# aminrezaee/mujoco_reinforcement_learning

Hardware: AMD Instinct MI355X
Metric: env-steps/sec (whole node) HalfCheetah-v4 4096 envs at 1/2/4/8 MI355X (higher is better)
Workload: dtype bf16; 1 GPU; HalfCheetah-v4 shapes: 4096 envs/GPU x 128 steps, obs 17, act 6, actor+critic 256x256 ReLU MLP, PPO 10 epochs x 8 minibatches of 65536; num_envs_per_gpu=4096, horizon=128, minibatch=65536, epochs=10, rng=philox, hipgraphs=True, env=device (synthetic dynamics on the GPU), parallelism=dp1 (env-sharded, RCCL grad all-reduce)

## Files before the change

### mujoco_reinforcement_learning_amd/csrc/fused_update.h

```cpp
#pragma once

#include <hip/hip_runtime.h>

#include <cstdint>

#include "ppo_loss.h"
#include "reduce_slabs.h"
#include "timing.h"

namespace ppo {

constexpr int kFusedRows = 64;
constexpr int kFusedKX = 32;
constexpr int kFusedSP = 16;
constexpr int kFusedMaxAct = 8;
constexpr int kFusedMaxWG = 128;
constexpr int kStampSlots = 13;

struct FusedNet {
  const __bf16 *w0b;
  const __bf16 *w1b;
  const __bf16 *w1bt;
  const float *w0, *w1;
  const float *b0, *b1;
  const float *wh, *bh;
  int64_t off_w0, off_b0, off_w1, off_b1, off_wh, off_bh;
};

constexpr int kRecordBytes = 2 * kFusedKX + 4 * kFusedSP;
static_assert(kRecordBytes == 128, "one record per 128 B line");
int fused_records_launch(uint4 *rec, const float *states, const float *actions,
                         const float *old_logp, const float *adv, const float *vtarget,
                         int64_t n_rows, int din, int act_dim, const TimRec &trec, hipStream_t st);

struct GaeRecordArgs {
  const float *value, *next_value;
  const void *reward;
  const uint8_t *done, *term;
  int force_last, n, t_len;
  float gamma_f, lg_f;
  float *adv, *vtarget;
  const float *states, *actions, *old_logp;
  uint4 *rec;
  int din, act_dim;
};
int gae_records_launch(const GaeRecordArgs &g, bool reward_f64, const TimRec &rec,
                       hipStream_t st);

struct AdamPackArgs {
  float *p;
  const float *g;
  float *m, *v;
  int64_t n, n_actor;
  const float *sched;
  float neg_a, neg_c, bc2;
  float w1, b2, omb2, eps;
  __bf16 *w0b[2], *w1b[2], *w1bt[2];
  int64_t off_w0[2], off_w1[2];
  int din, H;
};
int adam_pack_launch(const AdamPackArgs &a, const TimRec &rec, hipStream_t st);

struct TailArgs {
  AdamPackArgs a;
  const int32_t *rows;
  const uint4 *rec;
  int64_t n_rec;
  __bf16 *xb;
  float *srow;
  int b;
  bool reduce;
};
int step_tail_launch(const ReduceArgs &r, const TailArgs &t, const TimRec &rec, hipStream_t st);

struct FusedArgs {
  FusedNet net[2];
  const float *logstd;
  int64_t off_logstd;
  __bf16 *xb;
  float *srow;
  const float *states, *actions, *old_logp, *adv, *vtarget;
  const int32_t *rows;
  const int32_t *rows_n;
  const uint4 *rec;
  int64_t n_rec;
  bool direct;
  bool pack_w;
  int b, din, act_dim, act, hidden;
  float omv;
  LossCoef coef;
  float *slabs;
  int64_t slab_stride;
  float *loss_part;
  int G;
  uint64_t *stamps;
};
int fused_prep_launch(const FusedArgs &q, const TimRec &rec, hipStream_t st);
int fused_update_launch(const FusedArgs &q, const TimRec &rec, hipStream_t st);
bool fused_width_ok(int hidden);
int fused_sched(int act);

}
```

### mujoco_reinforcement_learning_amd/csrc/fused_update.hip

```cpp
#include <cstdio>
#include <cstdlib>
#include <type_traits>

#include "adam_elem.h"
#include "fused_common.h"
#include "gae_pipe.h"

namespace ppo {

using namespace fu;

__device__ __forceinline__ uint16_t bf16_bits(float x) { return static_cast<uint16_t>(pack2(x, 0.f) & 0xffffu); }

__global__ __launch_bounds__(256) void fused_prep_kernel(FusedArgs q, int row_blocks) {
  const int tid = threadIdx.x;
  if (static_cast<int>(blockIdx.x) < row_blocks && q.rec) {
    const int j = static_cast<int>((static_cast<int64_t>(blockIdx.x) * 256 + tid) >> 3);
    const int u = tid & 7;
    if (j >= q.b) return;
    const int count = q.rows_n ? *q.rows_n : q.b;
    uint4 v = make_uint4(0u, 0u, 0u, 0u);
    if (j < count) {
      const int64_t sr = q.rows[j];
      if (sr >= 0 && sr < q.n_rec) v = q.rec[sr * (kRecordBytes / 16) + u];
// ... 111 lines not shown
      s[k] = k < A ? act[b][k] : (k == A ? lp[b] : (k == A + 1 ? ad : (k == A + 2 ? vt : 0.f)));
    uint4 *d = rec + row * (kRecordBytes / 16);
#pragma unroll
    for (int u = 0; u < kFusedKX / 8; ++u)
      d[u] = make_uint4(pack2(x[b][8 * u], x[b][8 * u + 1]), pack2(x[b][8 * u + 2], x[b][8 * u + 3]),
                        pack2(x[b][8 * u + 4], x[b][8 * u + 5]), pack2(x[b][8 * u + 6], x[b][8 * u + 7]));
#pragma unroll
    for (int u = 0; u < kFusedSP / 4; ++u)
      d[kFusedKX / 8 + u] = make_uint4(__float_as_uint(s[4 * u]), __float_as_uint(s[4 * u + 1]),
                                       __float_as_uint(s[4 * u + 2]), __float_as_uint(s[4 * u + 3]));
  }
};

template <typename RT, int EB, int KMAX>
__global__ __launch_bounds__(EB * 16) void gae_records_kernel(GaeRecordArgs g) {
  RecordEmit em;
  em.states = g.states;
  em.actions = g.actions;
  em.old_logp = g.old_logp;
  em.rec = g.rec;
  em.din = g.din;
  em.A = g.act_dim;
  gae_pipe_body<RT, EB, KMAX>(g.value, g.next_value, static_cast<const RT *>(g.reward), g.done,
                              g.term, g.force_last, g.n, g.t_len, g.gamma_f, g.lg_f, g.adv,
                              g.vtarget, em);
}

constexpr int kPackTile = 32;

__global__ __launch_bounds__(256) void adam_pack_kernel(AdamPackArgs a, int gen_blocks) {
  const float ns_a = a.sched ? a.sched[0] : a.neg_a;
  const float ns_c = a.sched ? a.sched[1] : a.neg_c;
  const float bc2 = a.sched ? a.sched[2] : a.bc2;
  const int tid = threadIdx.x;
  const int H = a.H;
  if (static_cast<int>(blockIdx.x) < gen_blocks) {
    const int64_t i = static_cast<int64_t>(blockIdx.x) * 256 + tid;
    if (i >= a.n) return;
#pragma unroll
    for (int z = 0; z < 2; ++z)
      if (i >= a.off_w1[z] && i < a.off_w1[z] + static_cast<int64_t>(H) * H) return;
    float m = a.m[i], v = a.v[i];
    const float p = adam_elem(a.p[i], a.g[i], m, v, i < a.n_actor ? ns_a : ns_c, a.w1, a.b2,
                              a.omb2, bc2, a.eps);
    a.p[i] = p;
    a.m[i] = m;
    a.v[i] = v;
#pragma unroll
    for (int z = 0; z < 2; ++z) {
      const int64_t e = i - a.off_w0[z];
      if (e >= 0 && e < static_cast<int64_t>(H) * a.din) {
        const int f = static_cast<int>(e / a.din), k = static_cast<int>(e % a.din);
        reinterpret_cast<uint16_t *>(a.w0b[z])[f * kFusedKX + k] = bf16_bits(p);
      }
    }
    return;
  }
  __shared__ uint16_t tile[kPackTile][kPackTile + 2];
  const int tiles = H / kPackTile;
  const int tb = static_cast<int>(blockIdx.x) - gen_blocks;
  const int z = tb / (tiles * tiles);
  const int to = (tb % (tiles * tiles)) / tiles, tc = tb % tiles;
  const int64_t base = a.off_w1[z];
  const float ns = base < a.n_actor ? ns_a : ns_c;
  uint16_t *w1b = reinterpret_cast<uint16_t *>(a.w1b[z]);
  uint16_t *w1bt = reinterpret_cast<uint16_t *>(a.w1bt[z]);
#pragma unroll 4
  for (int k = 0; k < kPackTile * kPackTile / 256; ++k) {
    const int idx = k * 256 + tid, lo = idx / kPackTile, lc = idx % kPackTile;
    const int64_t t = static_cast<int64_t>(to * kPackTile + lo) * H + tc * kPackTile + lc;
    const int64_t i = base + t;
    float m = a.m[i], v = a.v[i];
    const float p = adam_elem(a.p[i], a.g[i], m, v, ns, a.w1, a.b2, a.omb2, bc2, a.eps);
    a.p[i] = p;
    a.m[i] = m;
    a.v[i] = v;
    const uint16_t hb = bf16_bits(p);
    w1b[w_frag(to * kPackTile + lo, tc * kPackTile + lc, H)] = hb;
    tile[lo][lc] = hb;
  }
  __syncthreads();
#pragma unroll 4
  for (int k = 0; k < kPackTile * kPackTile / 256; ++k) {
    const int idx = k * 256 + tid, lc = idx / kPackTile, lo = idx % kPackTile;
    w1bt[w_frag(tc * kPackTile + lc, to * kPackTile + lo, H)] = tile[lo][lc];
  }
}

__device__ __forceinline__ void tail_gather(const TailArgs &t, int64_t idx) {
  const int j = static_cast<int>(idx >> 3);
  const int u = static_cast<int>(idx & 7);
  if (j >= t.b) return;
  const int64_t sr = t.rows[j];
  uint4 v = make_uint4(0u, 0u, 0u, 0u);
  if (sr >= 0 && sr < t.n_rec) v = t.rec[sr * (kRecordBytes / 16) + u];
  if (u < 4) reinterpret_cast<uint4 *>(t.xb + static_cast<int64_t>(j) * kFusedKX)[u] = v;
  else reinterpret_cast<uint4 *>(t.srow + static_cast<int64_t>(j) * kFusedSP)[u - 4] = v;
}

__device__ __forceinline__ void adam_apply(const AdamPackArgs &a, int64_t i, float4 g4, float4 p4,
                                           float4 m4, float4 v4) {
  const float ns = i < a.n_actor ? (a.sched ? a.sched[0] : a.neg_a) : (a.sched ? a.sched[1] : a.neg_c);
  const float bc2 = a.sched ? a.sched[2] : a.bc2;
  p4.x = adam_elem(p4.x, g4.x, m4.x, v4.x, ns, a.w1, a.b2, a.omb2, bc2, a.eps);
  p4.y = adam_elem(p4.y, g4.y, m4.y, v4.y, ns, a.w1, a.b2, a.omb2, bc2, a.eps);
  p4.z = adam_elem(p4.z, g4.z, m4.z, v4.z, ns, a.w1, a.b2, a.omb2, bc2, a.eps);
  p4.w = adam_elem(p4.w, g4.w, m4.w, v4.w, ns, a.w1, a.b2, a.omb2, bc2, a.eps);
  *reinterpret_cast<float4 *>(a.p + i) = p4;
  *reinterpret_cast<float4 *>(a.m + i) = m4;
  *reinterpret_cast<float4 *>(a.v + i) = v4;
  const float pv[4] = {p4.x, p4.y, p4.z, p4.w};
  const int H = a.H;
#pragma unroll
  for (int z = 0; z < 2; ++z) {
    const int64_t e1 = i - a.off_w1[z];
    if (e1 >= 0 && e1 < static_cast<int64_t>(H) * H) {
      const int o = static_cast<int>(e1 / H), c = static_cast<int>(e1 % H);
      *reinterpret_cast<uint2 *>(a.w1b[z] + w_frag(o, c, H)) = make_uint2(pack2(pv[0], pv[1]), pack2(pv[2], pv[3]));
      uint16_t *wt = reinterpret_cast<uint16_t *>(a.w1bt[z]);
#pragma unroll
      for (int e = 0; e < 4; ++e) wt[w_frag(c + e, o, H)] = bf16_bits(pv[e]);
    }
    const int64_t e0 = i - a.off_w0[z];
#pragma unroll
    for (int e = 0; e < 4; ++e) {
      if (e0 + e >= 0 && e0 + e < static_cast<int64_t>(H) * a.din) {
        const int f = static_cast<int>((e0 + e) / a.din), k = static_cast<int>((e0 + e) % a.din);
        reinterpret_cast<uint16_t *>(a.w0b[z])[f * kFusedKX + k] = bf16_bits(pv[e]);
      }
    }
  }
}

template <int G>
__device__ __forceinline__ void tail_block(const ReduceArgs &r, const TailArgs &t, int64_t blk,
                                           RedScratch sc) {
  const int tid = threadIdx.x;
  const AdamPackArgs &a = t.a;
  const int64_t i = blk * (4 * G) + 4 * (tid % G);
  const bool lead = tid < G;
  float4 g4;
  if (t.reduce) {
    g4 = reduce_slab_block_s<G>(r, blk, sc);
    if (!lead || i >= r.total) return;
  } else {
    if (!lead || i >= a.n) return;
    g4 = *reinterpret_cast<const float4 *>(a.g + i);
  }
  adam_apply(a, i, g4, *reinterpret_cast<const float4 *>(a.p + i),
             *reinterpret_cast<const float4 *>(a.m + i), *reinterpret_cast<const float4 *>(a.v + i));
}

template <int G>
__global__ __launch_bounds__(G * kRedChunks) void step_tail_kernel(ReduceArgs r, TailArgs t, int red_blocks) {
  __shared__ __attribute__((aligned(16))) char scratch[red_scratch_bytes<G>()];
  constexpr int NT = G * kRedChunks;
  const int tid = threadIdx.x;
  if (static_cast<int>(blockIdx.x) >= red_blocks) {
    tail_gather(t, (static_cast<int64_t>(blockIdx.x) - red_blocks) * NT + tid);
    return;
  }
  tail_block<G>(r, t, blockIdx.x, red_scratch<G>(scratch));
}

template <int H, bool F32A2>
struct Lds {
  static constexpr int PITCH = 2 * H;
  static constexpr int A2P = 4 * H + 16;
  static constexpr int WHB = 0;
  static constexpr int BIAS = WHB + HeadImg<H>::BYTES;
  static constexpr int X = BIAS + 2 * H * 4;
  static constexpr int A1 = X + R * 64;
  static constexpr int D2 = A1 + R * PITCH;
  static constexpr int A2 = D2 + R * PITCH;
  static constexpr int A2BYTES = F32A2 ? R * A2P : R * PITCH;
  static constexpr int DZ = A2 + A2BYTES;
  static constexpr int DZT = DZ + R * kDzRowBytes;
  static constexpr int HS = DZT + 16 * kDzTPitch;
  static constexpr int SROW = HS + 80 * 4;
  static constexpr int RED = SROW;
  static constexpr int W0 = SROW + R * kFusedSP * 4;
  static constexpr int WHT = W0 + (F32A2 ? 0 : H * 64);
  static constexpr int X2 = WHT + (F32A2 ? 0 : H * 32);
  static constexpr int TOTAL = X2 + (F32A2 ? 0 : R * 64);
  static_assert(TOTAL <= 163840, "LDS budget");
  static_assert(R * PITCH <= A2BYTES, "D1 image must fit in the a2 region");
};


__device__ __forceinline__ bf16x8 pack8(float4 u, float4 v) {
  const uint4 p = make_uint4(pack2(u.x, u.y), pack2(u.z, u.w), pack2(v.x, v.y), pack2(v.z, v.w));
  return __builtin_bit_cast(bf16x8, p);
}

__device__ __forceinline__ void mfma16_drain(f32x4 &acc) { asm volatile("s_nop 15" : "+v"(acc)); }


template <int H, int ACT, int NH, bool ACTOR, bool STAMP, int SCHED>
__device__ __forceinline__ void fused_body(const FusedArgs &q, const FusedNet &N, char *lds,
                                           uint64_t *stamps) {
  static_assert(H == 32 * NW, "wave w owns feature tile w");
  constexpr bool F32A2 = ACT != PPO_ACT_RELU;
  constexpr bool DEFER_DW0 = (SCHED & 1) && !F32A2;
  bool have_prev = false;
  using L = Lds<H, F32A2>;
  constexpr int z = ACTOR ? 0 : 1;
  char *ximg = lds + L::X;
  char *xprev = lds + L::X2;
  char *const a1img = lds + L::A1;
  char *const d2img = lds + L::D2;
  char *const a2img = lds + L::A2;
  char *const d1img = lds + L::A2;
  char *const whb = lds + L::WHB;
  char *const dzimg = lds + L::DZ;
  char *const dztimg = lds + L::DZT;
  const float *const b0s = reinterpret_cast<const float *>(lds + L::BIAS);
  const float *const b1s = b0s + H;
  const float *const a2f = reinterpret_cast<const float *>(lds + L::A2);

  const int tid0 = threadIdx.x, w = tid0 >> 6;
  int tid = tid0, lane = tid & 63, r = lane & 31, h = lane >> 5;
#define OPAQUE_LANE()             \
  tid = tid0;                     \
  asm volatile("" : "+v"(tid));   \
  lane = tid & 63;                \
  r = lane & 31;                  \
  h = lane >> 5
  const int A = q.act_dim;
  const int G = q.G;
  const int nchunks = (q.b + R - 1) / R;
  const int count = q.rows_n ? *q.rows_n : q.b;

  const char *const rbase = q.direct ? reinterpret_cast<const char *>(q.rec)
                                     : reinterpret_cast<const char *>(q.xb);
  const int rshift = q.direct ? 7 : 6;
  const int64_t rhi = q.direct ? 64
                               : reinterpret_cast<const char *>(q.srow) - reinterpret_cast<const char *>(q.xb);
  const int rlast = static_cast<int>(min(q.n_rec, static_cast<int64_t>(INT32_MAX)) - 1);
  auto row_index = [&](int c) -> int {
    const int j = min(c * R + (tid0 >> 3), q.b - 1);
    return *gptr(q.rows + j);
  };
  auto row_ok = [&](int c, int sr, int t) -> bool {
    const int j = c * R + (t >> 3);
    return j < q.b && j < count && (!q.direct || (sr >= 0 && sr <= rlast));
  };
  auto load_half = [&](int c, int sr, int t, bool scalars) -> uint64_t {
    const int j = c * R + (t >> 3);
    const int row = q.direct ? min(max(sr, 0), rlast) : min(j, q.b - 1);
    const int64_t off = (static_cast<int64_t>(row) << rshift) + 8 * (t & 7) + (scalars ? rhi : 0);
    return *gptr(reinterpret_cast<const uint64_t *>(rbase + off));
  };
  const int i_first = row_index(blockIdx.x);

  uint64_t t_body0 = 0, t_real0 = 0;
  if constexpr (STAMP) {
    t_body0 = __builtin_amdgcn_s_memtime();
    t_real0 = __builtin_amdgcn_s_memrealtime();
    __builtin_amdgcn_s_waitcnt(0xC07F);
  }
  stage_head_image<H>(whb, N.wh, ACTOR ? A : 1, tid, NT);
  for (int i = tid; i < 2 * H; i += NT) {
    const float *b = i < H ? N.b0 : N.b1;
    (reinterpret_cast<float *>(lds + L::BIAS))[i] = b ? b[i % H] : 0.f;
  }
  if (tid < 32) {
    const int a = tid & 15;
    const bool ok = a < (ACTOR ? A : 1);
    (reinterpret_cast<float *>(lds + L::HS))[tid] =
        tid < 16 ? ((ok && N.bh) ? N.bh[a] : 0.f) : ((ACTOR && ok) ? q.logstd[a] : 0.f);
  }
  if (tid < 16) {
    const bool ok = ACTOR && tid < A;
    const float sd = ok ? expf(q.logstd[tid]) : 1.f;
    const float var = sd * sd;
    (reinterpret_cast<float *>(lds + L::HS))[32 + tid] = ok ? logf(sd) : 0.f;
    (reinterpret_cast<float *>(lds + L::HS))[48 + tid] = 1.f / var;
    (reinterpret_cast<float *>(lds + L::HS))[64 + tid] = 1.f / (2.f * var);
  }
  if constexpr (!F32A2) {
    for (int i = tid; i < H * 4; i += NT) {
      const uint4 v = reinterpret_cast<const uint4 *>(N.w0b)[i];
      *reinterpret_cast<uint4 *>(lds + L::W0 + x_off(i >> 2, i & 3)) = v;
    }
    const int nh_real = ACTOR ? A : 1;
    for (int i = tid; i < H * 16; i += NT) {
      const int a = i / H, f = i % H;
      const float v = a < nh_real ? N.wh[a * H + f] : 0.f;
      *reinterpret_cast<uint16_t *>(lds + L::WHT + 2 * (f * 16 + a)) = bf16_bits(v);
    }
  }
  const float *const hbias = reinterpret_cast<const float *>(lds + L::HS);
  uint64_t xpre = load_half(blockIdx.x, i_first, tid0, false);
  bool xok = row_ok(blockIdx.x, i_first, tid0);
  if constexpr (DEFER_DW0) {
    for (int i = tid; i < R * (2 * H) / 16; i += NT)
      *reinterpret_cast<uint4 *>(lds + L::A2 + 16 * i) = make_uint4(0u, 0u, 0u, 0u);
    for (int i = tid; i < R * 64 / 16; i += NT)
      *reinterpret_cast<uint4 *>(lds + L::X + 16 * i) = make_uint4(0u, 0u, 0u, 0u);
  }
  lds_sync();

  f32x16 gw1[2][4];
  f32x16 gw0;
#pragma unroll
  for (int a = 0; a < 2; ++a)
#pragma unroll
    for (int b = 0; b < 4; ++b)
#pragma unroll
      for (int e = 0; e < 16; ++e) gw1[a][b][e] = 0.f;
#pragma unroll
  for (int e = 0; e < 16; ++e) gw0[e] = 0.f;
  f32x4 ghw[2];
#pragma unroll
  for (int u = 0; u < 2; ++u) ghw[u] = f32x4{0.f, 0.f, 0.f, 0.f};
// ... 388 lines not shown
  tid = tid0;
  lane = tid & 63;
  r = lane & 31;
  h = lane >> 5;
  if constexpr (STAMP) t_prev = __builtin_amdgcn_s_memtime();
  float *slab = q.slabs + static_cast<int64_t>(blockIdx.x) * q.slab_stride;
#pragma unroll
  for (int a = 0; a < 2; ++a)
#pragma unroll
    for (int b = 0; b < 4; ++b) {
      const int o0 = 32 * (2 * (w & 3) + a), i0 = 32 * (4 * (w >> 2) + b);
#pragma unroll
      for (int e = 0; e < 16; ++e)
        slab[N.off_w1 + static_cast<int64_t>(o0 + reg_feature(e, h)) * H + i0 + r] = gw1[a][b][e];
    }
  if (r < q.din) {
#pragma unroll
    for (int e = 0; e < 16; ++e)
      slab[N.off_w0 + static_cast<int64_t>(32 * w + reg_feature(e, h)) * q.din + r] = gw0[e];
  }
  if ((lane & 1) == 0) {
    const int f = 32 * w + rs16_feature(lane);
    if (N.b1) slab[N.off_b1 + f] = gb1;
    if (N.b0) slab[N.off_b0 + f] = gb0;
  }
  const int na = ACTOR ? A : 1;
#pragma unroll
  for (int u = 0; u < 2; ++u)
#pragma unroll
    for (int i = 0; i < 4; ++i) {
      const int a = 4 * (lane >> 4) + i;
      if (a < na) slab[N.off_wh + static_cast<int64_t>(a) * H + 32 * w + 16 * u + (lane & 15)] = ghw[u][i];
    }
  float *red = reinterpret_cast<float *>(lds + L::RED);
  {
    g_bh += __shfl_xor(g_bh, 16, 64);
    g_bh += __shfl_xor(g_bh, 32, 64);
    g_ls += __shfl_xor(g_ls, 16, 64);
    g_ls += __shfl_xor(g_ls, 32, 64);
    g_loss += __shfl_xor(g_loss, 16, 64);
    g_loss += __shfl_xor(g_loss, 32, 64);
    if (lane < 16) {
      float *dst = red + (w * 16 + lane) * 4;
      dst[0] = g_bh;
      dst[1] = g_ls;
      dst[2] = g_loss;
    }
  }
  lds_sync();
  if (tid < na) {
    float sb = 0.f, sl = 0.f;
#pragma unroll
    for (int v = 0; v < NW; ++v) {
      sb += red[(v * 16 + tid) * 4];
      sl += red[(v * 16 + tid) * 4 + 1];
    }
    if (N.bh) slab[N.off_bh + tid] = sb;
    if (ACTOR) slab[q.off_logstd + tid] = sl;
  }
  if (tid == 0) {
    float s = 0.f;
#pragma unroll
    for (int v = 0; v < NW; ++v) s += red[(v * 16) * 4 + 2];
    q.loss_part[2 * blockIdx.x + z] = s;
  }
  if constexpr (STAMP) {
    __builtin_amdgcn_s_waitcnt(0);
    __syncthreads();
    const uint64_t t_end = __builtin_amdgcn_s_memtime();
    const uint64_t r_end = __builtin_amdgcn_s_memrealtime();
    __builtin_amdgcn_s_waitcnt(0xC07F);
    t_acc[11] = t_end - t_prev;
    t_acc[12] = r_end - t_real0;
    if (tid0 == 0) {
      uint64_t *dst = stamps + (static_cast<int64_t>(z) * gridDim.x + blockIdx.x) * kStampSlots;
#pragma unroll
      for (int p = 0; p < kStampSlots; ++p) dst[p] = t_acc[p];
    }
  }
}

template <int H, int ACT, int NA, bool STAMP, int SCHED = 0>
__global__ __launch_bounds__(NT, 1) void fused_update_kernel(FusedArgs q, uint64_t *stamps) {
  __shared__ __attribute__((aligned(16))) char lds[Lds<H, ACT != PPO_ACT_RELU>::TOTAL];
  if (blockIdx.y == 0) fused_body<H, ACT, NA, true, STAMP, SCHED>(q, q.net[0], lds, stamps);
  else fused_body<H, ACT, 1, false, STAMP, SCHED>(q, q.net[1], lds, stamps);
}

bool fused_width_ok(int hidden) { return hidden == 256; }

int fused_prep_launch(const FusedArgs &q, const TimRec &rec, hipStream_t st) {
  const int row_blocks = q.rec ? static_cast<int>(ceil_div(static_cast<int64_t>(q.b) * 8, 256))
                               : ceil_div(q.b, 256);
  const int64_t per_net = static_cast<int64_t>(q.hidden) * (kFusedKX + q.hidden);
  const int w_blocks = q.pack_w ? static_cast<int>(ceil_div(2 * per_net, 256)) : 0;
  if (row_blocks + w_blocks == 0) return 0;
  launch_k(rec, fused_prep_kernel, dim3(row_blocks + w_blocks), dim3(256), 0, st, q, row_blocks);
  PPO_LAUNCHED();
  return 0;
}

int fused_records_launch(uint4 *rec, const float *states, const float *actions,
                         const float *old_logp, const float *adv, const float *vtarget,
                         int64_t n_rows, int din, int act_dim, const TimRec &trec, hipStream_t st) {
  PPO_REQUIRE(din >= 1 && din <= kFusedKX && act_dim >= 1 && act_dim + 3 <= kFusedSP,
              "fused records: din %d / act_dim %d out of range", din, act_dim);
  if (n_rows <= 0) return 0;
  launch_k(trec, fused_records_kernel, dim3(ceil_div(n_rows, 256)), dim3(256), 0, st, rec, states,
           actions, old_logp, adv, vtarget, n_rows, din, act_dim);
  PPO_LAUNCHED();
  return 0;
}

int gae_records_launch(const GaeRecordArgs &g, bool reward_f64, const TimRec &rec,
                       hipStream_t st) {
  PPO_REQUIRE(g.din >= 1 && g.din <= kFusedKX && g.act_dim >= 1 && g.act_dim + 3 <= kFusedSP &&
                  g.n > 0 && g.t_len > 0 && g.t_len <= 16 * 16,
              "gae_records: din %d / act_dim %d / n %d / t %d out of range", g.din, g.act_dim, g.n,
              g.t_len);
  auto go = [&](auto rt_tag, auto eb_tag, auto k_tag) {
    using RT = decltype(rt_tag);
    constexpr int EB = decltype(eb_tag)::value, KM = decltype(k_tag)::value;
    TimRec r = rec;
    if (tim_active())
      r.name = intern_name("gae_records_kernel<%s, %d, %d>", sizeof(RT) == 8 ? "double" : "float",
                           EB, KM);
    launch_k(r, gae_records_kernel<RT, EB, KM>, dim3(ceil_div(g.n, EB)), dim3(EB * 16), 0, st, g);
  };
  auto by_k = [&](auto rt_tag, auto eb_tag) {
    if (g.t_len <= 16 * 8) go(rt_tag, eb_tag, std::integral_constant<int, 8>{});
    else go(rt_tag, eb_tag, std::integral_constant<int, 16>{});
  };
  auto by_eb = [&](auto rt_tag) {
    if (g.n >= 16384) by_k(rt_tag, std::integral_constant<int, 32>{});
    else by_k(rt_tag, std::integral_constant<int, 16>{});
  };
  if (reward_f64) by_eb(double{});
  else by_eb(float{});
  PPO_LAUNCHED();
  return 0;
}

int adam_pack_launch(const AdamPackArgs &a, const TimRec &rec, hipStream_t st) {
  PPO_REQUIRE(a.H % kPackTile == 0 && a.din >= 1 && a.din <= kFusedKX && a.n > 0,
              "adam_pack: H=%d din=%d", a.H, a.din);
  const int gen_blocks = static_cast<int>(ceil_div(a.n, 256));
  const int tiles = a.H / kPackTile;
  launch_k(rec, adam_pack_kernel, dim3(gen_blocks + 2 * tiles * tiles), dim3(256), 0, st, a,
           gen_blocks);
  PPO_LAUNCHED();
  return 0;
}

static const int g_tail_groups = [] {
  const char *v = getenv("PPO_TAIL_GROUPS");
  return v ? atoi(v) : 32;
}();

int step_tail_launch(const ReduceArgs &r, const TailArgs &t, const TimRec &rec, hipStream_t st) {
  PPO_REQUIRE(t.a.H % 4 == 0 && t.a.din >= 1 && t.a.din <= kFusedKX &&
                  (!t.reduce || r.total == t.a.n),
              "step tail: H=%d din=%d", t.a.H, t.a.din);
  auto go = [&](auto gc) {
    constexpr int G = decltype(gc)::value, NT = G * kRedChunks;
    const int red_blocks = static_cast<int>(ceil_div(t.a.n, 4 * G));
    const int gather_blocks = static_cast<int>(ceil_div(static_cast<int64_t>(t.b) * 8, NT));
    TimRec named = rec;
    if (tim_active()) named.name = intern_name("step_tail_kernel<%d>", G);
    launch_k(named, step_tail_kernel<G>, dim3(red_blocks + gather_blocks), dim3(NT), 0, st, r, t,
             red_blocks);
  };
  if (g_tail_groups == 8) go(std::integral_constant<int, 8>{});
  else if (g_tail_groups == 16) go(std::integral_constant<int, 16>{});
  else go(std::integral_constant<int, 32>{});
  PPO_LAUNCHED();
  return 0;
}

static int env_fused_sched() {
  const char *v = getenv("PPO_FUSED_SCHED");
  return v ? atoi(v) : 1;
}

int fused_sched(int act) {
  const int s = env_fused_sched();
  return act == PPO_ACT_RELU && s == 1 ? 1 : 0;
}

template <int ACT, int NA, int SCHED>
static void launch_sched(const FusedArgs &q, const TimRec &rec, hipStream_t st) {
  uint64_t *nul = nullptr;
  if (ACT == PPO_ACT_RELU && q.stamps)
    launch_k(rec, fused_update_kernel<256, ACT, NA, true, SCHED>, dim3(q.G, 2), dim3(NT), 0, st, q, q.stamps);
  else
    launch_k(rec, fused_update_kernel<256, ACT, NA, false, SCHED>, dim3(q.G, 2), dim3(NT), 0, st, q, nul);
}

template <int ACT, int NA>
static void launch_na(const FusedArgs &q, const TimRec &rec, hipStream_t st) {
  if constexpr (ACT == PPO_ACT_RELU) {
    const int sched = fused_sched(ACT);
    if (sched == 1) return launch_sched<ACT, NA, 1>(q, rec, st);
  }
  launch_sched<ACT, NA, 0>(q, rec, st);
}

template <int ACT>
static void launch_act(const FusedArgs &q, const TimRec &rec, hipStream_t st) {
  if (q.act_dim <= 2) launch_na<ACT, 2>(q, rec, st);
  else if (q.act_dim <= 4) launch_na<ACT, 4>(q, rec, st);
  else if (q.act_dim <= 6) launch_na<ACT, 6>(q, rec, st);
  else launch_na<ACT, 8>(q, rec, st);
}

int fused_update_launch(const FusedArgs &q, const TimRec &rec, hipStream_t st) {
  PPO_REQUIRE(q.hidden == 256, "fused update: hidden width %d not compiled", q.hidden);
  PPO_REQUIRE(q.G >= 1 && q.G <= kFusedMaxWG, "fused update: bad workgroup count %d", q.G);
  PPO_REQUIRE(q.act_dim >= 1 && q.act_dim <= kFusedMaxAct, "fused update: act_dim %d", q.act_dim);
  PPO_REQUIRE(!q.stamps || q.act == PPO_ACT_RELU, "fused update: phase stamps only for ReLU");
  PPO_REQUIRE(q.rows && q.b > 0 && (!q.direct || (q.rec && q.n_rec > 0)),
              "fused update: rows / records missing (b=%d, direct=%d)", q.b, int(q.direct));
  if (q.act == PPO_ACT_RELU) launch_act<PPO_ACT_RELU>(q, rec, st);
  else if (q.act == PPO_ACT_TANH) launch_act<PPO_ACT_TANH>(q, rec, st);
  else launch_act<PPO_ACT_ELU>(q, rec, st);
  PPO_LAUNCHED();
  return 0;
}

}
```

### mujoco_reinforcement_learning_amd/csrc/mlp_engine.hip

```cpp
#include <algorithm>
#include <cstdarg>
#include <cstdio>
#include <cstdlib>
#include <cstring>
#include <deque>
#include <mutex>
#include <new>
#include <string>
#include <type_traits>
#include <vector>

#include "common.h"
#include "ctx.h"
#include "fused_policy.h"
#include "fused_update.h"
#include "gemm.h"
#include "gemm_ops.h"
#include "ppo_loss.h"
#include "reduce_slabs.h"
#include "timing.h"
#include "wide_path.h"

namespace ppo {

// ... 1137 lines not shown
  g.term = terminated_d;
  g.force_last = force_last_done;
  g.n = n;
  g.t_len = t;
  g.gamma_f = static_cast<float>(gamma);
  g.lg_f = static_cast<float>(lmbda * gamma);
  g.adv = adv_d;
  g.vtarget = vtarget_d;
  g.states = states_d;
  g.actions = actions_d;
  g.old_logp = old_logp_d;
  g.rec = ctx->frec;
  g.din = din;
  g.act_dim = A;
  const double per_row = 4 + 4 + (reward_is_f64 ? 8 : 4) + 1 + (done_d ? 1 : 0) + 4 + 4 +
                         4.0 * (din + A + 1) + kRecordBytes;
  const TimRec rec{KC_GAE, "gae_records_kernel", 0.0, static_cast<double>(n_rows) * per_row};
  return gae_records_launch(g, reward_is_f64 != 0, rec, st);
}

extern "C" int ppo_minibatch_grad_staged(ppo_ctx *ctx, const int32_t *rows_d, int b,
                                         const int32_t *count_d, float clip_lo, float clip_hi,
                                         float entropy_coef, float inv_b, float inv_ba,
                                         float *grad_d, float *loss_d, int flags, void *stream) {
  if (int rc = check_ctx(ctx)) return rc;
  PPO_REQUIRE(fused_active(ctx) && ctx->frec && ctx->frec_rows > 0,
              "ppo_minibatch_grad_staged: no staged records (ppo_stage_records first)");
  PPO_REQUIRE(rows_d && grad_d && loss_d, "ppo_minibatch_grad_staged: null buffer");
  PPO_REQUIRE(b > 0 && b <= ctx->cfg.max_rows,
              "ppo_minibatch_grad_staged: b=%d outside [1, max_rows=%d]", b, ctx->cfg.max_rows);
  PPO_REQUIRE((flags & ~(PPO_STAGED_WEIGHTS_CURRENT | PPO_STAGED_ROWS_GATHERED)) == 0,
              "ppo_minibatch_grad_staged: flags %d", flags);
  PPO_REQUIRE(!(flags & PPO_STAGED_ROWS_GATHERED) || count_d == nullptr,
              "ppo_minibatch_grad_staged: pre-gathered rows take no device count");
  TimingScope timing_scope(ctx);
  return fused_minibatch_grad(ctx, nullptr, nullptr, nullptr, nullptr, nullptr, rows_d, b,
                              count_d, LossCoef{clip_lo, clip_hi, entropy_coef, inv_b, inv_ba},
                              grad_d, loss_d, as_stream(stream), true,
                              (flags & PPO_STAGED_WEIGHTS_CURRENT) == 0,
                              (flags & PPO_STAGED_ROWS_GATHERED) != 0);
}

extern "C" int ppo_adam_pack_gather(ppo_ctx *ctx, const float *g_d, float *m_d, float *v_d,
                                    const float *sched_d, float neg_step_actor,
                                    float neg_step_critic, float bc2_sqrt, float one_minus_beta1,
                                    float beta2, float one_minus_beta2, float eps,
                                    const int32_t *next_rows_d, int next_b, void *stream) {
  if (int rc = check_ctx(ctx)) return rc;
  PPO_REQUIRE(fused_active(ctx) && ctx->frec && ctx->frec_rows > 0,
              "ppo_adam_pack_gather: no staged records (ppo_stage_records first)");
  PPO_REQUIRE(g_d && m_d && v_d, "ppo_adam_pack_gather: null buffer");
  PPO_REQUIRE(next_b >= 0 && next_b <= ctx->cfg.max_rows && (next_b == 0) == (next_rows_d == nullptr),
              "ppo_adam_pack_gather: next_b=%d", next_b);
  TimingScope timing_scope(ctx);
  TailArgs t{};
  t.a = adam_pack_args(ctx, g_d, m_d, v_d, sched_d, neg_step_actor, neg_step_critic, bc2_sqrt,
                       one_minus_beta1, beta2, one_minus_beta2, eps);
  t.rows = next_rows_d;
  t.rec = ctx->frec;
  t.n_rec = ctx->frec_rows;
  t.xb = ctx->fxb;
  t.srow = ctx->fsrow;
  const bool direct = next_b > 0 && fused_args(ctx, nullptr, nullptr, nullptr, nullptr, nullptr,
                                               next_rows_d, next_b, nullptr, LossCoef{}, true,
                                               false).direct;
  t.b = direct ? 0 : next_b;
  t.reduce = false;
  ReduceArgs r{};
  r.total = ctx->total_params;
  const double P = static_cast<double>(ctx->total_params), H = ctx->fused_hidden;
  const TimRec rec{KC_ADAM, "step_tail_kernel", 0.0,
                   28.0 * P + 2.0 * 2.0 * H * (t.a.din + 2.0 * H) +
                       static_cast<double>(t.b) * (4.0 + 2.0 * kRecordBytes)};
  if (int rc = step_tail_launch(r, t, rec, as_stream(stream))) {
    note_gathered(ctx, nullptr, 0);
    return rc;
  }
  if (t.b > 0) note_gathered(ctx, next_rows_d, t.b);
  return 0;
}

extern "C" int ppo_gather_staged_rows(ppo_ctx *ctx, const int32_t *rows_d, int b, void *stream) {
  if (int rc = check_ctx(ctx)) return rc;
  PPO_REQUIRE(fused_active(ctx) && ctx->frec && ctx->frec_rows > 0,
              "ppo_gather_staged_rows: no staged records (ppo_stage_records first)");
  PPO_REQUIRE(rows_d && b > 0 && b <= ctx->cfg.max_rows,
              "ppo_gather_staged_rows: b=%d outside [1, max_rows=%d]", b, ctx->cfg.max_rows);
  TimingScope timing_scope(ctx);
  const FusedArgs q = fused_args(ctx, nullptr, nullptr, nullptr, nullptr, nullptr, rows_d, b,
                                 nullptr, LossCoef{}, true, false);
  if (int rc = fused_prep(ctx, q, as_stream(stream))) return rc;
  note_gathered(ctx, rows_d, b);
  return 0;
}

extern "C" int ppo_adam_pack(ppo_ctx *ctx, const float *g_d, float *m_d, float *v_d,
                             const float *sched_d, float neg_step_actor, float neg_step_critic,
                             float bc2_sqrt, float one_minus_beta1, float beta2,
                             float one_minus_beta2, float eps, void *stream) {
  if (int rc = check_ctx(ctx)) return rc;
  PPO_REQUIRE(fused_active(ctx), "ppo_adam_pack: needs the fused bf16 path");
  PPO_REQUIRE(g_d && m_d && v_d, "ppo_adam_pack: null buffer");
  TimingScope timing_scope(ctx);
  const AdamPackArgs a = adam_pack_args(ctx, g_d, m_d, v_d, sched_d, neg_step_actor,
                                        neg_step_critic, bc2_sqrt, one_minus_beta1, beta2,
                                        one_minus_beta2, eps);
  const double Hd = a.H;
  const TimRec rec{KC_ADAM, "adam_pack_kernel", 0.0,
                   28.0 * a.n + 2.0 * 2.0 * Hd * (a.din + 2.0 * Hd)};
  return adam_pack_launch(a, rec, as_stream(stream));
}

extern "C" int ppo_update_step_staged(ppo_ctx *ctx, const int32_t *rows_d, int b,
                                      const int32_t *next_rows_d, int next_b, float clip_lo,
                                      float clip_hi, float entropy_coef, float inv_b,
                                      float inv_ba, float *grad_d, float *loss_d, float *m_d,
                                      float *v_d, const float *sched_d, float neg_step_actor,
                                      float neg_step_critic, float bc2_sqrt,
                                      float one_minus_beta1, float beta2, float one_minus_beta2,
                                      float eps, int flags, void *stream) {
  if (int rc = check_ctx(ctx)) return rc;
  PPO_REQUIRE(fused_active(ctx) && ctx->frec && ctx->frec_rows > 0,
              "ppo_update_step_staged: no staged records (ppo_stage_records first)");
  PPO_REQUIRE(rows_d && grad_d && loss_d && m_d && v_d, "ppo_update_step_staged: null buffer");
  PPO_REQUIRE(b > 0 && b <= ctx->cfg.max_rows && next_b >= 0 && next_b <= ctx->cfg.max_rows &&
                  (next_b == 0) == (next_rows_d == nullptr),
              "ppo_update_step_staged: b=%d next_b=%d (max_rows %d)", b, next_b,
              ctx->cfg.max_rows);
  PPO_REQUIRE((flags & ~(PPO_STAGED_WEIGHTS_CURRENT | PPO_STAGED_ROWS_GATHERED)) == 0,
              "ppo_update_step_staged: flags %d", flags);
  hipStream_t st = as_stream(stream);
  TimingScope timing_scope(ctx);
  const bool gathered = (flags & PPO_STAGED_ROWS_GATHERED) && gathered_holds(ctx, rows_d, b);
  const bool current = flags & PPO_STAGED_WEIGHTS_CURRENT;
  FusedArgs q = fused_args(ctx, nullptr, nullptr, nullptr, nullptr, nullptr, rows_d, b, nullptr,
                           LossCoef{clip_lo, clip_hi, entropy_coef, inv_b, inv_ba}, true, !current);
  if ((!gathered && !q.direct) || !current) {
    FusedArgs p = q;
    p.b = (gathered || q.direct) ? 0 : b;
    if (int rc = fused_prep(ctx, p, st)) return rc;
    if (p.b > 0) note_gathered(ctx, rows_d, b);
  }
  const ReduceArgs r = fused_reduce_args(ctx, q, grad_d, loss_d);
  TailArgs t{};
  t.a = adam_pack_args(ctx, grad_d, m_d, v_d, sched_d, neg_step_actor, neg_step_critic, bc2_sqrt,
                       one_minus_beta1, beta2, one_minus_beta2, eps);
  t.rows = next_rows_d;
  t.rec = ctx->frec;
  t.n_rec = ctx->frec_rows;
  t.xb = ctx->fxb;
  t.srow = ctx->fsrow;
  t.b = q.direct ? 0 : next_b;
  t.reduce = true;
  if (int rc = fused_forward_backward(ctx, q, st)) {
    note_gathered(ctx, nullptr, 0);
    return rc;
  }
  const double P = static_cast<double>(ctx->total_params), H = ctx->fused_hidden;
  const TimRec rec{KC_REDUCE, "step_tail_kernel", static_cast<double>(q.G) * P,
                   4.0 * (q.G + 1.0) * P + 24.0 * P + 2.0 * 2.0 * H * (q.din + 2.0 * H) +
                       static_cast<double>(t.b) * (4.0 + 2.0 * kRecordBytes)};
  if (int rc = step_tail_launch(r, t, rec, st)) {
    note_gathered(ctx, nullptr, 0);
    return rc;
  }
  if (t.b > 0) note_gathered(ctx, next_rows_d, t.b);
  return 0;
}

extern "C" int ppo_observe_act(ppo_ctx *ctx, double *window_d, const double *obs_d,
                               const uint8_t *reset_d, int all_reset, const int32_t *bounds,
                               int n_bounds, int normalize, float *state_d, int n,
                               const float *eps_d, uint64_t seed, uint64_t offset,
                               float *action_d, float *logp_d, float *value_d, float *mean_d,
                               void *stream) {
  if (int rc = check_ctx(ctx)) return rc;
  const int o = ctx->cfg.obs_dim, w = ctx->cfg.window;
  PPO_REQUIRE(window_d && state_d && n > 0, "ppo_observe_act: null window/state or n <= 0");
  PPO_REQUIRE(n <= ctx->cfg.max_rows, "ppo_observe_act: n=%d exceeds max_rows=%d", n,
              ctx->cfg.max_rows);
  PPO_REQUIRE(n_bounds >= 0 && n_bounds < 16, "ppo_observe_act: too many slices (%d)", n_bounds);
  PolicySlices tab{};
  tab.count = normalize ? n_bounds : 0;
  for (int i = 0; i <= n_bounds && normalize; ++i) {
    PPO_REQUIRE(bounds != nullptr, "ppo_observe_act: null bounds");
    PPO_REQUIRE(bounds[i] >= 0 && bounds[i] <= o && (i == 0 || bounds[i] >= bounds[i - 1]),
                "ppo_observe_act: bounds must be ascending within [0, O]");
    tab.edge[i] = bounds[i];
  }
  if (!fused_active(ctx) && wide_active(ctx) && wide_observe_ok(ctx, tab.count)) {
    TimingScope timing_scope(ctx);
    if (int rc = wide_observe(ctx, window_d, obs_d, reset_d, all_reset, tab, normalize, state_d, n,
                              as_stream(stream)))
      return rc;
    return wide_policy_step(ctx, state_d, n, eps_d, seed, offset, action_d, logp_d, value_d,
                            mean_d, false, as_stream(stream), true);
  }
  if (!fused_active(ctx) || w > kPolicyMaxWindow) {
    if (obs_d) {
      int rc = ppo_obs_window_push(window_d, obs_d, 1, reset_d, all_reset, n, o, w, stream);
      if (rc) return rc;
    }
    if (int rc = ppo_obs_normalize(window_d, state_d, n, o, w, bounds, n_bounds, normalize, stream))
      return rc;
    if (wide_active(ctx)) {
      TimingScope timing_scope(ctx);
      return wide_policy_step(ctx, state_d, n, eps_d, seed, offset, action_d, logp_d, value_d,
                              mean_d, false, as_stream(stream));
    }
    return ppo_policy_step(ctx, state_d, n, eps_d, seed, offset, action_d, logp_d, value_d,
                           mean_d, stream);
  }
  TimingScope timing_scope(ctx);
  PolicyFusedArgs q{};
  fused_nets(ctx, q.net);
  q.logstd = ctx->params + ctx->net[0].logstd_off;
  q.n = n;
  q.obs_dim = o;
  q.window = w;
  q.act_dim = ctx->cfg.act_dim;
  q.act = ctx->cfg.activation;
  q.hidden = ctx->fused_hidden;
  q.omv = ctx->cfg.output_max_value;
  q.window_d = window_d;
  q.obs_d = obs_d;
  q.reset_d = reset_d;
  q.all_reset = all_reset;
  q.tab = tab;
  q.normalize = normalize;
  q.state_d = state_d;
  q.do_actor = (action_d || logp_d || mean_d) ? 1 : 0;
  q.do_critic = value_d ? 1 : 0;
  q.eps = eps_d;
  q.seed = seed;
  q.offset = offset;
  q.offset_base = ctx->rng_counter;
  q.stamps = ctx->fstamp_on ? ctx->fstamps : nullptr;
  if (q.stamps) ctx->fstamp_g = 128;
  q.action = action_d;
  q.logp = logp_d;
  q.value = value_d;
  q.mean = mean_d;
  const double H = ctx->fused_hidden, A = ctx->cfg.act_dim, din = o * w;
  const double fl = 2.0 * n * ((q.do_actor ? din * H + H * H + A * H : 0.0) +
                               (q.do_critic ? din * H + H * H + H : 0.0));
  const double by = static_cast<double>(n) *
                    (8.0 * o * w * (obs_d ? 2.0 : 1.0) + (obs_d ? 8.0 * o : 0.0) + 4.0 * din +
                     (eps_d ? 4.0 * A : 0.0) + (action_d ? 4.0 * A : 0.0) + (mean_d ? 4.0 * A : 0.0) +
                     (logp_d ? 4.0 : 0.0) + (value_d ? 4.0 : 0.0));
  const TimRec rec{KC_POLICY_HEAD,
                   tim_active() ? intern_name("policy_fused_kernel<%d, %d, %d, false>", ctx->fused_hidden, q.act,
                                             q.act_dim <= 2 ? 2 : q.act_dim <= 4 ? 4 : q.act_dim <= 6 ? 6 : 8)
                                : nullptr,
                   fl, by};
  return policy_fused_launch(q, rec, as_stream(stream));
}

extern "C" int ppo_minibatch_grad(ppo_ctx *ctx, const float *states_d, const float *actions_d,
                                  const float *old_logp_d, const float *adv_d,
                                  const float *vtarget_d, const int32_t *rows_d, int b,
                                  const int32_t *count_d, float clip_lo, float clip_hi,
                                  float entropy_coef, float inv_b, float inv_ba, float *grad_d,
                                  float *loss_d, void *stream) {
  if (int rc = check_ctx(ctx)) return rc;
  PPO_REQUIRE(states_d && actions_d && old_logp_d && adv_d && vtarget_d && rows_d && grad_d,
              "ppo_minibatch_grad: null buffer");
  PPO_REQUIRE(b > 0 && b <= ctx->cfg.max_rows, "ppo_minibatch_grad: b=%d outside [1, max_rows=%d]",
              b, ctx->cfg.max_rows);
  const LossCoef coef{clip_lo, clip_hi, entropy_coef, inv_b, inv_ba};
  hipStream_t st = as_stream(stream);
  TimingScope timing_scope(ctx);
  if (fused_active(ctx))
    return fused_minibatch_grad(ctx, states_d, actions_d, old_logp_d, adv_d, vtarget_d, rows_d, b,
                                count_d, coef, grad_d, loss_d, st);
  if (wide_active(ctx))
    return wide_minibatch_grad(ctx, states_d, actions_d, old_logp_d, adv_d, vtarget_d, rows_d, b,
                               count_d, coef, grad_d, loss_d, st);
  const bool both[2] = {true, true};
  const int din = ctx->cfg.obs_dim * ctx->cfg.window;
  const int A = ctx->cfg.act_dim;
  launch_k(TimRec{KC_GATHER, "gather_states_kernel", 0.0, 4.0 * b * (2.0 * din + 1)},
           gather_states_kernel, dim3(ceil_div(static_cast<int64_t>(b) * ctx->ldx, 256)),
           dim3(256), 0, st, states_d, rows_d, count_d, b, din, ctx->ldx, ctx->xg);
  PPO_LAUNCHED();
  if (int rc = forward_hidden(ctx, both, ctx->xg, nullptr, b, count_d, st, ctx->ldx)) return rc;

  NetDesc &NA = ctx->net[0], &NC = ctx->net[1];
  const LayerDesc &HA = NA.layer[NA.n_hidden], &HC = NC.layer[NC.n_hidden];
  int head_splits = std::min(kHeadSplits, std::max(1, b / 32));
  UpdateHeadArgs u{};
  u.ha = NA.h[NA.n_hidden - 1];
  u.hc = NC.h[NC.n_hidden - 1];
  u.ga = NA.g;
  u.gc = NC.g;
  u.dza = NA.dz;
  u.dzc = NC.dz;
  u.da = HA.in;
  u.dc = HC.in;
  u.act_dim = A;
  u.act = ctx->cfg.activation;
  u.wa = ctx->params + HA.w_off;
  u.ba = HA.b_off >= 0 ? ctx->params + HA.b_off : nullptr;
  u.logstd = ctx->params + NA.logstd_off;
  u.wc = ctx->params + HC.w_off;
  u.bc = ctx->params + HC.b_off;
  u.omv = ctx->cfg.output_max_value;
// ... 348 lines not shown
```

### mujoco_reinforcement_learning_amd/csrc/reduce_slabs.h

```cpp
#pragma once

#include <hip/hip_runtime.h>

#include <cstdint>

#include "common.h"

namespace ppo {

constexpr int kMaxSegs = 48;
struct ReduceSeg {
  int64_t dst, len;
  const float *src;
  int64_t stride;
  int nsplit;
};
struct ReduceArgs {
  ReduceSeg seg[kMaxSegs];
  int nseg;
  int64_t total;
  float *grad;
  const float *loss_part;
  int loss_splits;
  float inv_b;
  const float *logstd;
  int act_dim;
  float ent_coef;
  float *loss_out;
};

constexpr int kRedGroups = 32;
constexpr int kRedChunks = 16;
constexpr int kRedThreads = kRedGroups * kRedChunks;
constexpr int kRedParams = 4 * kRedGroups;
constexpr int kLossSlots = 512;
struct RedScratch {
  float4 *part;
  float *lred;
  ReduceSeg *sseg;
};
template <int G = kRedGroups>
constexpr int red_scratch_bytes() {
  return (kRedChunks * G) * 16 + 2 * kLossSlots * 4 + kMaxSegs * static_cast<int>(sizeof(ReduceSeg));
}
constexpr int kRedScratchBytes = red_scratch_bytes<kRedGroups>();
template <int G = kRedGroups>
__device__ __forceinline__ RedScratch red_scratch(char *lds) {
  return RedScratch{reinterpret_cast<float4 *>(lds),
                    reinterpret_cast<float *>(lds + kRedChunks * G * 16),
                    reinterpret_cast<ReduceSeg *>(lds + kRedChunks * G * 16 + 2 * kLossSlots * 4)};
}

__device__ __forceinline__ int seg_find(const ReduceSeg *sseg, int nseg, int64_t i) {
  int s = 0, hi = nseg - 1;
  while (s < hi) {
    const int mid = (s + hi + 1) >> 1;
    if (sseg[mid].dst <= i) s = mid;
    else hi = mid - 1;
  }
  return s;
}

__device__ __forceinline__ float4 slab_item_sum(const ReduceArgs &q, const ReduceSeg *sseg,
                                                int64_t i, int chunk) {
  float4 acc = make_float4(0.f, 0.f, 0.f, 0.f);
  if (i >= q.total) return acc;
  const ReduceSeg &g = sseg[seg_find(sseg, q.nseg, i)];
  const int64_t off = i - g.dst;
  const int k0 = (g.nsplit * chunk) / kRedChunks, k1 = (g.nsplit * (chunk + 1)) / kRedChunks;
  if (off >= 0 && off + 3 < g.len && g.stride % 4 == 0 &&
      reinterpret_cast<uintptr_t>(g.src) % 16 == 0) {
    const float *src = g.src + off;
    float4 acc1 = make_float4(0.f, 0.f, 0.f, 0.f);
    int k = k0;
#pragma unroll 4
    for (; k + 1 < k1; k += 2) {
      const float4 v = *reinterpret_cast<const float4 *>(src + k * g.stride);
      const float4 u = *reinterpret_cast<const float4 *>(src + (k + 1) * g.stride);
      acc.x += v.x;
      acc.y += v.y;
      acc.z += v.z;
      acc.w += v.w;
      acc1.x += u.x;
      acc1.y += u.y;
      acc1.z += u.z;
      acc1.w += u.w;
    }
    if (k < k1) {
      const float4 v = *reinterpret_cast<const float4 *>(src + k * g.stride);
      acc.x += v.x;
      acc.y += v.y;
      acc.z += v.z;
      acc.w += v.w;
    }
    acc = make_float4(acc.x + acc1.x, acc.y + acc1.y, acc.z + acc1.z, acc.w + acc1.w);
  } else if (off >= 0) {
    float a4[4] = {0.f, 0.f, 0.f, 0.f};
#pragma unroll
    for (int e = 0; e < 4; ++e) {
      if (off + e >= g.len) continue;
      const float *src = g.src + off + e;
      float s[8] = {0.f, 0.f, 0.f, 0.f, 0.f, 0.f, 0.f, 0.f};
      int k = k0;
      for (; k + 7 < k1; k += 8) {
#pragma unroll
        for (int j = 0; j < 8; ++j) s[j] += src[static_cast<int64_t>(k + j) * g.stride];
      }
      for (; k < k1; ++k) s[0] += src[static_cast<int64_t>(k) * g.stride];
      a4[e] = ((s[0] + s[1]) + (s[2] + s[3])) + ((s[4] + s[5]) + (s[6] + s[7]));
    }
    acc = make_float4(a4[0], a4[1], a4[2], a4[3]);
  }
  return acc;
}

__device__ __forceinline__ float4 chunk_combine(const float4 *part, int stride, int grp) {
  float4 out = part[grp];
#pragma unroll
  for (int c = 1; c < kRedChunks; ++c) {
    const float4 b = part[c * stride + grp];
    out = make_float4(out.x + b.x, out.y + b.y, out.z + b.z, out.w + b.w);
  }
  return out;
}

template <int NT = kRedThreads>
__device__ __forceinline__ void reduce_loss_block(const ReduceArgs &q, float *lred_flat) {
  static_assert(kLossSlots % NT == 0, "loss slots per thread");
  float (*lred)[kLossSlots] = reinterpret_cast<float (*)[kLossSlots]>(lred_flat);
  const int tid = threadIdx.x;
  for (int v = tid; v < kLossSlots; v += NT) {
    float la = 0.f, lc = 0.f;
    for (int k = v; k < q.loss_splits; k += kLossSlots) {
      la += q.loss_part[2 * k];
      lc += q.loss_part[2 * k + 1];
    }
    lred[0][v] = la;
    lred[1][v] = lc;
  }
  __syncthreads();
  for (int w = kLossSlots / 2; w > 0; w >>= 1) {
    for (int v = tid; v < w; v += NT) {
      lred[0][v] += lred[0][v + w];
      lred[1][v] += lred[1][v + w];
    }
    __syncthreads();
  }
  if (tid == 0) {
    float h = 0.f;
    if (q.logstd) {
      for (int a = 0; a < q.act_dim; ++a) h += kEntropyConst + logf(expf(q.logstd[a]));
      h = h / static_cast<float>(q.act_dim);
    }
    q.loss_out[0] = -(lred[0][0] * q.inv_b) - h * q.ent_coef;
    q.loss_out[1] = lred[1][0] * q.inv_b;
  }
}

template <int G = kRedGroups>
__device__ __forceinline__ float4 reduce_slab_block_s(const ReduceArgs &q, int64_t block,
                                                      RedScratch sc) {
  const int tid = threadIdx.x, grp = tid % G, chunk = tid / G;
  const int64_t i = block * (4 * G) + 4 * grp;
  if (tid < q.nseg) sc.sseg[tid] = q.seg[tid];
  __syncthreads();
  sc.part[chunk * G + grp] = slab_item_sum(q, sc.sseg, i, chunk);
  __syncthreads();
  float4 out = make_float4(0.f, 0.f, 0.f, 0.f);
  if (chunk == 0 && i < q.total) {
    out = chunk_combine(sc.part, G, grp);
    *reinterpret_cast<float4 *>(q.grad + i) = out;
  }
  if (block == 0 && q.loss_out) reduce_loss_block<G * kRedChunks>(q, sc.lred);
  return out;
}

__device__ __forceinline__ float4 reduce_slab_block(const ReduceArgs &q, int64_t block) {
  __shared__ __attribute__((aligned(16))) char scratch[kRedScratchBytes];
  return reduce_slab_block_s(q, block, red_scratch(scratch));
}

}
```

Baseline: 52.88 million env-steps/s.

## Add fast path in step tail for interior w1 blocks with per-element Adam and bf16 pack

Splits the step-tail grid into slow, gather and fast blocks. Fast blocks cover the aligned interior of each network's hidden-hidden weight matrix and skip the generic segment lookup. They spread the Adam update across all 4G lead threads per element, then write the bf16 transposed and fragment-packed weight copies directly, using lane shuffles to pack 8 values per store. It also drops the env-selectable group count in favour of a fixed kRedGroups, and moves the aligned slab sum into a shared helper. The change adds index-remapping logic and relies on the segment layout matching the expected w1 region; if it does not, it falls back to the generic path.

```diff
diff --git a/mujoco_reinforcement_learning_amd/csrc/fused_update.h b/mujoco_reinforcement_learning_amd/csrc/fused_update.h
--- a/mujoco_reinforcement_learning_amd/csrc/fused_update.h
+++ b/mujoco_reinforcement_learning_amd/csrc/fused_update.h
@@ -70,6 +70,10 @@
   float *srow;
   int b;
   bool reduce;
+  const float *slabs;
+  int64_t slab_stride;
+  int nsplit;
+  int fast_lo[2], fast_hi[2];
 };
 int step_tail_launch(const ReduceArgs &r, const TailArgs &t, const TimRec &rec, hipStream_t st);
 
diff --git a/mujoco_reinforcement_learning_amd/csrc/fused_update.hip b/mujoco_reinforcement_learning_amd/csrc/fused_update.hip
--- a/mujoco_reinforcement_learning_amd/csrc/fused_update.hip
+++ b/mujoco_reinforcement_learning_amd/csrc/fused_update.hip
@@ -287,15 +287,70 @@
 }
 
 template <int G>
-__global__ __launch_bounds__(G * kRedChunks) void step_tail_kernel(ReduceArgs r, TailArgs t, int red_blocks) {
+__device__ __forceinline__ void tail_fast(const ReduceArgs &r, const TailArgs &t, int j, char *lds) {
+  constexpr int NP = 4 * G;
+  static_assert(NP % 64 == 0, "the lead threads fill whole waves (lane shuffles)");
+  const AdamPackArgs &a = t.a;
+  const int tid = threadIdx.x, grp = tid % G, chunk = tid / G;
+  const bool lead = tid < NP;
+  const int n0 = t.fast_hi[0] - t.fast_lo[0], z = j >= n0 ? 1 : 0;
+  const int k0 = (t.nsplit * chunk) / kRedChunks, k1 = (t.nsplit * (chunk + 1)) / kRedChunks;
+  const int64_t i0 = static_cast<int64_t>(z == 0 ? t.fast_lo[0] + j : t.fast_lo[1] + (j - n0)) * NP;
+  const int64_t i = i0 + tid;
+  float p = 0.f, m = 0.f, v = 0.f;
+  if (lead) {
+    p = a.p[i];
+    m = a.m[i];
+    v = a.v[i];
+  }
+  float4 *part = reinterpret_cast<float4 *>(lds);
+  part[chunk * G + grp] = slab_sum_aligned(t.slabs + i0 + 4 * grp, t.slab_stride, k0, k1);
+  lds_sync();
+  if (!lead) return;
+  const float *pf = reinterpret_cast<const float *>(part);
+  float g = pf[tid];
+#pragma unroll
+  for (int c = 1; c < kRedChunks; ++c) g += pf[c * NP + tid];
+  r.grad[i] = g;
+  const float ns = z == 0 ? (a.sched ? a.sched[0] : a.neg_a) : (a.sched ? a.sched[1] : a.neg_c);
+  const float bc2 = a.sched ? a.sched[2] : a.bc2;
+  p = adam_elem(p, g, m, v, ns, a.w1, a.b2, a.omb2, bc2, a.eps);
+  a.p[i] = p;
+  a.m[i] = m;
+  a.v[i] = v;
+  const int H = a.H;
+  const uint32_t e1 = static_cast<uint32_t>(i - a.off_w1[z]);
+  const int o = static_cast<int>(e1 / static_cast<uint32_t>(H));
+  const int c = static_cast<int>(e1 % static_cast<uint32_t>(H));
+  const uint32_t hb = bf16_bits(p);
+  reinterpret_cast<uint16_t *>(a.w1bt[z])[w_frag(c, o, H)] = static_cast<uint16_t>(hb);
+  const uint32_t pair = hb | (static_cast<uint32_t>(__shfl_down(static_cast<int>(hb), 1)) << 16);
+  const uint32_t q1 = static_cast<uint32_t>(__shfl_down(static_cast<int>(pair), 2));
+  const uint32_t q2 = static_cast<uint32_t>(__shfl_down(static_cast<int>(pair), 4));
+  const uint32_t q3 = static_cast<uint32_t>(__shfl_down(static_cast<int>(pair), 6));
+  if ((tid & 7) == 0)
+    *reinterpret_cast<uint4 *>(a.w1b[z] + w_frag(o, c, H)) = make_uint4(pair, q1, q2, q3);
+}
+
+template <int G>
+__global__ __launch_bounds__(G * kRedChunks) void step_tail_kernel(ReduceArgs r, TailArgs t,
+                                                                    int slow_blocks, int gather_blocks) {
   __shared__ __attribute__((aligned(16))) char scratch[red_scratch_bytes<G>()];
   constexpr int NT = G * kRedChunks;
   const int tid = threadIdx.x;
-  if (static_cast<int>(blockIdx.x) >= red_blocks) {
-    tail_gather(t, (static_cast<int64_t>(blockIdx.x) - red_blocks) * NT + tid);
+  int bid = blockIdx.x;
+  if (bid < slow_blocks) {
+    if (bid >= t.fast_lo[0]) bid += t.fast_hi[0] - t.fast_lo[0];
+    if (bid >= t.fast_lo[1]) bid += t.fast_hi[1] - t.fast_lo[1];
+    tail_block<G>(r, t, bid, red_scratch<G>(scratch));
     return;
   }
-  tail_block<G>(r, t, blockIdx.x, red_scratch<G>(scratch));
+  bid -= slow_blocks;
+  if (bid < gather_blocks) {
+    tail_gather(t, static_cast<int64_t>(bid) * NT + tid);
+    return;
+  }
+  tail_fast<G>(r, t, bid - gather_blocks, scratch);
 }
 
 template <int H, bool F32A2>
@@ -990,27 +1045,45 @@
   return 0;
 }
 
-static const int g_tail_groups = [] {
-  const char *v = getenv("PPO_TAIL_GROUPS");
-  return v ? atoi(v) : 32;
-}();
-
-int step_tail_launch(const ReduceArgs &r, const TailArgs &t, const TimRec &rec, hipStream_t st) {
-  PPO_REQUIRE(t.a.H % 4 == 0 && t.a.din >= 1 && t.a.din <= kFusedKX &&
-                  (!t.reduce || r.total == t.a.n),
-              "step tail: H=%d din=%d", t.a.H, t.a.din);
-  auto go = [&](auto gc) {
-    constexpr int G = decltype(gc)::value, NT = G * kRedChunks;
-    const int red_blocks = static_cast<int>(ceil_div(t.a.n, 4 * G));
-    const int gather_blocks = static_cast<int>(ceil_div(static_cast<int64_t>(t.b) * 8, NT));
-    TimRec named = rec;
-    if (tim_active()) named.name = intern_name("step_tail_kernel<%d>", G);
-    launch_k(named, step_tail_kernel<G>, dim3(red_blocks + gather_blocks), dim3(NT), 0, st, r, t,
-             red_blocks);
-  };
-  if (g_tail_groups == 8) go(std::integral_constant<int, 8>{});
-  else if (g_tail_groups == 16) go(std::integral_constant<int, 16>{});
-  else go(std::integral_constant<int, 32>{});
+static void mark_interior(const ReduceArgs &r, TailArgs &t, int np) {
+  for (int z = 0; z < 2; ++z) t.fast_lo[z] = t.fast_hi[z] = 0;
+  if (!t.reduce || !t.slabs || t.slab_stride % 4 != 0 || t.nsplit < 1 || t.a.H % 8 != 0 ||
+      reinterpret_cast<uintptr_t>(t.slabs) % 16 != 0)
+    return;
+  int64_t prev_hi = 1;
+  for (int z = 0; z < 2; ++z) {
+    const int64_t off = t.a.off_w1[z], len = static_cast<int64_t>(t.a.H) * t.a.H;
+    bool ok = false;
+    for (int s = 0; s < r.nseg; ++s) {
+      const ReduceSeg &g = r.seg[s];
+      ok = ok || (g.dst == off && g.len == len && g.src == t.slabs + off &&
+                  g.stride == t.slab_stride && g.nsplit == t.nsplit);
+    }
+    const int64_t lo = std::max<int64_t>(prev_hi, ceil_div(off, np)), hi = (off + len) / np;
+    if (!ok || off % 8 != 0 || lo >= hi) {
+      t.fast_lo[z] = t.fast_hi[z] = static_cast<int>(prev_hi);
+      continue;
+    }
+    t.fast_lo[z] = static_cast<int>(lo);
+    t.fast_hi[z] = static_cast<int>(hi);
+    prev_hi = hi;
+  }
+}
+
+int step_tail_launch(const ReduceArgs &r, const TailArgs &t_in, const TimRec &rec, hipStream_t st) {
+  PPO_REQUIRE(t_in.a.H % 4 == 0 && t_in.a.din >= 1 && t_in.a.din <= kFusedKX &&
+                  (!t_in.reduce || r.total == t_in.a.n),
+              "step tail: H=%d din=%d", t_in.a.H, t_in.a.din);
+  constexpr int G = kRedGroups, NT = G * kRedChunks;
+  TailArgs t = t_in;
+  mark_interior(r, t, 4 * G);
+  const int n_fast = (t.fast_hi[0] - t.fast_lo[0]) + (t.fast_hi[1] - t.fast_lo[1]);
+  const int slow_blocks = static_cast<int>(ceil_div(t.a.n, 4 * G)) - n_fast;
+  const int gather_blocks = static_cast<int>(ceil_div(static_cast<int64_t>(t.b) * 8, NT));
+  TimRec named = rec;
+  if (tim_active()) named.name = intern_name("step_tail_kernel<%d>", G);
+  launch_k(named, step_tail_kernel<G>, dim3(slow_blocks + gather_blocks + n_fast), dim3(NT), 0, st,
+           r, t, slow_blocks, gather_blocks);
   PPO_LAUNCHED();
   return 0;
 }
diff --git a/mujoco_reinforcement_learning_amd/csrc/mlp_engine.hip b/mujoco_reinforcement_learning_amd/csrc/mlp_engine.hip
--- a/mujoco_reinforcement_learning_amd/csrc/mlp_engine.hip
+++ b/mujoco_reinforcement_learning_amd/csrc/mlp_engine.hip
@@ -1313,6 +1313,9 @@
   t.srow = ctx->fsrow;
   t.b = q.direct ? 0 : next_b;
   t.reduce = true;
+  t.slabs = ctx->fslabs;
+  t.slab_stride = ctx->total_params;
+  t.nsplit = q.G;
   if (int rc = fused_forward_backward(ctx, q, st)) {
     note_gathered(ctx, nullptr, 0);
     return rc;
diff --git a/mujoco_reinforcement_learning_amd/csrc/reduce_slabs.h b/mujoco_reinforcement_learning_amd/csrc/reduce_slabs.h
--- a/mujoco_reinforcement_learning_amd/csrc/reduce_slabs.h
+++ b/mujoco_reinforcement_learning_amd/csrc/reduce_slabs.h
@@ -61,6 +61,34 @@
   return s;
 }
 
+__device__ __forceinline__ float4 slab_sum_aligned(const float *src, int64_t stride, int k0,
+                                                   int k1) {
+  float4 acc = make_float4(0.f, 0.f, 0.f, 0.f);
+  float4 acc1 = make_float4(0.f, 0.f, 0.f, 0.f);
+  int k = k0;
+#pragma unroll 4
+  for (; k + 1 < k1; k += 2) {
+    const float4 v = *reinterpret_cast<const float4 *>(src + k * stride);
+    const float4 u = *reinterpret_cast<const float4 *>(src + (k + 1) * stride);
+    acc.x += v.x;
+    acc.y += v.y;
+    acc.z += v.z;
+    acc.w += v.w;
+    acc1.x += u.x;
+    acc1.y += u.y;
+    acc1.z += u.z;
+    acc1.w += u.w;
+  }
+  if (k < k1) {
+    const float4 v = *reinterpret_cast<const float4 *>(src + k * stride);
+    acc.x += v.x;
+    acc.y += v.y;
+    acc.z += v.z;
+    acc.w += v.w;
+  }
+  return make_float4(acc.x + acc1.x, acc.y + acc1.y, acc.z + acc1.z, acc.w + acc1.w);
+}
+
 __device__ __forceinline__ float4 slab_item_sum(const ReduceArgs &q, const ReduceSeg *sseg,
                                                 int64_t i, int chunk) {
   float4 acc = make_float4(0.f, 0.f, 0.f, 0.f);
@@ -70,30 +98,7 @@
   const int k0 = (g.nsplit * chunk) / kRedChunks, k1 = (g.nsplit * (chunk + 1)) / kRedChunks;
   if (off >= 0 && off + 3 < g.len && g.stride % 4 == 0 &&
       reinterpret_cast<uintptr_t>(g.src) % 16 == 0) {
-    const float *src = g.src + off;
-    float4 acc1 = make_float4(0.f, 0.f, 0.f, 0.f);
-    int k = k0;
-#pragma unroll 4
-    for (; k + 1 < k1; k += 2) {
-      const float4 v = *reinterpret_cast<const float4 *>(src + k * g.stride);
-      const float4 u = *reinterpret_cast<const float4 *>(src + (k + 1) * g.stride);
-      acc.x += v.x;
-      acc.y += v.y;
-      acc.z += v.z;
-      acc.w += v.w;
-      acc1.x += u.x;
-      acc1.y += u.y;
-      acc1.z += u.z;
-      acc1.w += u.w;
-    }
-    if (k < k1) {
-      const float4 v = *reinterpret_cast<const float4 *>(src + k * g.stride);
-      acc.x += v.x;
-      acc.y += v.y;
-      acc.z += v.z;
-      acc.w += v.w;
-    }
-    acc = make_float4(acc.x + acc1.x, acc.y + acc1.y, acc.z + acc1.z, acc.w + acc1.w);
+    acc = slab_sum_aligned(g.src + off, g.stride, k0, k1);
   } else if (off >= 0) {
     float a4[4] = {0.f, 0.f, 0.f, 0.f};
 #pragma unroll
```

After: 53.62 million env-steps/s, median of 6. 1.4% higher.
